# StanfordASL/RiskAverseTrajOpt

Hardware: AMD Instinct MI355X
Metric: SAA constraint-eval throughput (higher is better)
Workload: dtype f32

## Files before the change

### include/rato_saa.h

```cpp
#ifndef RATO_SAA_H
#define RATO_SAA_H

#include <stddef.h>
#include <stdint.h>

#ifdef __cplusplus
extern "C" {
#endif

#define RATO_OK 0
#define RATO_EINVAL (-1)
#define RATO_ENONFINITE (-2)
#define RATO_EINFEASIBLE (-4)
#define RATO_ENOCOMM (-3)
#define RATO_ERANK (-6)
#define RATO_ESELECT (-7)
#define RATO_ENNLS (-8)
#define RATO_EHIP (-1000)
#define RATO_ERCCL (-2000)

#define RATO_TILE 256
#define RATO_DRONE_NOBS 3
#define RATO_HOPPER_NFEAT 30

// ... 147 lines not shown
int rato_hopper_slip_host_inputs(int32_t M, int32_t C, const float* px_host, const float* fx_host,
                                 const float* fz_host, const float* a, const float* theta, const float* tau,
                                 const float* lam, float* Z, float* h, float* dh_dfz, float* dh_dpx,
                                 float* part_hess, void* stream);

int rato_hopper_slip_hessian(int32_t M, int32_t C, const float* px, const float* fx, const float* fz,
                             int32_t host_inputs, const float* a, const float* theta, const float* tau,
                             const float* lam, float* Z, float* h, float* dh_dfz, float* dh_dpx, float* part_hess3,
                             void* stream);

int64_t rato_hopper_jacobian_nnz(int32_t M, int32_t C, int32_t saa);
int rato_hopper_emit_jacobian_values(int32_t M, int32_t C, int32_t saa, double alpha, const float* dh_dfz,
                                     const float* dh_dpx, const float* chain_host, const float* chain_dev,
                                     int32_t write_constants, float* out, void* stream);


int rato_emit_csc_values(const float* G, const float* W ,
                         int64_t ld , int32_t tile, int32_t n_g, int32_t R, int32_t S,
                         int64_t M, float scale, float* out, void* stream);


int rato_saa_rowmax(const float* G, const float* W ,
                    int32_t tile, int32_t R, int32_t S, int64_t M, int64_t ld,
                    const float* base, double sign , const double* xs, int32_t n_u,
                    float* m_out, int32_t* arg_out, void* stream);

int rato_drone_rowmax_implicit(const rato_drone_params* p, const float* mass, const float* A22,
                               int32_t a22_axes ,
                               const float* W, const float* base, double sign, const double* xs,
                               float* m_out, int32_t* arg_out, void* stream);

int rato_drone_linearize_generators(const rato_drone_params* p, const float* us, const float* dW,
                                    const float* mass, const float* Qsym,
                                    float* A22, float* W, float* g_up, float* Z, float* part, void* stream);

int rato_saa_tail_rows_batch(const float* G, const float* W , int64_t ld, int32_t tile,
                             int32_t R, int32_t S, int64_t M, const float* base,
                             const float* m_base, const int32_t* arg_base, const double* stats_base,
                             int64_t stats_stride, const int32_t* slots, int32_t K, double alphaM, double* part,
                             void* stream);

int rato_drone_tail_rows_implicit(const rato_drone_params* p, const float* mass, const float* A22, int32_t a22_axes,
                                  const float* W, const float* base,
                                  const float* m_base, const int32_t* arg_base, const double* stats_base,
                                  int64_t stats_stride, const int32_t* slots, int32_t K, double alphaM,
                                  double* part, void* stream);

int rato_drone_rowmax_rollout(const rato_drone_params* p, const double* uk, const float* dW, const float* mass,
                              const float* Qsym, const double* xs, float* m_out, int32_t* arg_out, void* stream);
int rato_drone_tail_rows_rollout(const rato_drone_params* p, const double* uk, const float* dW, const float* mass,
                                 const float* Qsym, const float* m_base, const int32_t* arg_base,
                                 const double* stats_base, int64_t stats_stride, const int32_t* slots, int32_t K,
                                 double alphaM, double* part, void* stream);

int rato_car_rowmax_rollout(const rato_car_params* p, const double* uk, const float* dW, const float* x0_ped,
                            const float* w_speed, const float* w_rep, const double* xs, float* m_out,
                            int32_t* arg_out, void* stream);
int rato_car_tail_rows_rollout(const rato_car_params* p, const double* uk, const float* dW, const float* x0_ped,
                               const float* w_speed, const float* w_rep, const float* m_base, const int32_t* arg_base,
                               const double* stats_base, int64_t stats_stride, const int32_t* slots, int32_t K,
                               double alphaM, double* part, void* stream);

int rato_cut_oracle_rollout(int32_t system, const void* params, const double* uk, const float* s0, const float* s1,
                            const float* s2, const float* s3, const double* x_host, double* x_dev, float* m_out,
                            int32_t* arg_out, double alpha, float thr, double alphaM, void* workspace,
                            size_t workspace_bytes, double* res_dev, double* part_dev, double* res_host, void* stream);

int rato_kkt_sums(const float* m_star, int64_t M, const float* m_base, const double* stats_base, int64_t stats_stride,
                  const int32_t* slots, const double* lam, int32_t K, double alphaM, double v, double* part, void* stream);

typedef struct {
  int32_t system, S, cap, keep_max, keep_recent, keep_idle, mode_saa, recycle;
  int64_t M;
  double alpha, alphaM, c_s, rhs0, u_min, u_max;
  float thr;
  const void* params;
  const float *s0, *s1, *s2, *s3;
  double *uk_dev, *uk_host, *x_host, *x_dev;
  float* ring_m;
  int32_t* ring_arg;
  double* ring_res;
  void* workspace;
  size_t workspace_bytes;
  double *part, *part_b, *sums_b_host;
  int32_t *slots_dev, *slots_host;
  double* res_host;
  const double *p_diag, *q;
} rato_cut_config;

typedef struct {
  double* us;
  double slack, t_risk, phi, oracle_s, master_s, lam_slack;
  int32_t cuts, recycled, status, uncertified_cuts;
  int32_t* cut_slot;
  double* cut_lambda;
  int32_t cut_capacity, n_cut_rows;
  int32_t* bound_var;
  double* bound_sign;
  double* bound_lambda;
  int32_t bound_capacity, n_bounds;
} rato_cut_result;

typedef struct rato_cut_solver rato_cut_solver;
int rato_cut_solver_create(rato_cut_solver** out, const rato_cut_config* cfg);
void rato_cut_solver_destroy(rato_cut_solver* s);
size_t rato_cut_config_bytes(void);
// ... 281 lines not shown
```

### riskaversetrajopt_amd/_lib.py

```python
import ctypes as C
import os

from . import _build

_LIB = None
ABI_VERSION = 12

c_float_p = C.c_void_p
c_stream = C.c_void_p


class DroneParams(C.Structure):
    _fields_ = [("M", C.c_int32), ("ld", C.c_int32), ("S", C.c_int32), ("dt", C.c_float), ("beta", C.c_float),
                ("drag", C.c_float), ("kp", C.c_float), ("kd", C.c_float), ("tol", C.c_float),
                ("x_init", C.c_float * 6), ("x_final", C.c_float * 6),
                ("obs_xy", (C.c_float * 2) * 3), ("rows_out", C.c_int32),
                ("dt64", C.c_double), ("beta64", C.c_double), ("drag64", C.c_double), ("kp64", C.c_double),
                ("kd64", C.c_double), ("tol64", C.c_double), ("x_init64", C.c_double * 6),
                ("x_final64", C.c_double * 6), ("obs_xy64", (C.c_double * 2) * 3),
                ("stats_workspace", C.c_void_p), ("stats_out", C.c_void_p), ("stats_alpha", C.c_double),
                ("stats_thr", C.c_float), ("stats_flags", C.c_int32)]


class CarParams(C.Structure):
# ... 31 lines not shown
    _fields_ = [(k, C.c_int32) for k in ("n_tiles", "per_cu", "slots", "qslots", "wants_queue", "form", "split", "n_whole",
                                         "workgroups", "n_units")]


class CutConfig(C.Structure):
    _fields_ = [(k, C.c_int32) for k in ("system", "S", "cap", "keep_max", "keep_recent", "keep_idle", "mode_saa",
                                         "recycle")] + \
               [("M", C.c_int64)] + [(k, C.c_double) for k in ("alpha", "alphaM", "c_s", "rhs0", "u_min", "u_max")] + \
               [("thr", C.c_float), ("params", C.c_void_p)] + [(k, C.c_void_p) for k in ("s0", "s1", "s2", "s3")] + \
               [(k, C.c_void_p) for k in ("uk_dev", "uk_host", "x_host", "x_dev", "ring_m", "ring_arg", "ring_res",
                                          "workspace")] + [("workspace_bytes", C.c_size_t)] + \
               [(k, C.c_void_p) for k in ("part", "part_b", "sums_b_host", "slots_dev", "slots_host", "res_host",
                                          "p_diag", "q")]


class CutResult(C.Structure):
    _fields_ = [("us", C.c_void_p)] + \
               [(k, C.c_double) for k in ("slack", "t_risk", "phi", "oracle_s", "master_s", "lam_slack")] + \
               [(k, C.c_int32) for k in ("cuts", "recycled", "status", "uncertified_cuts")] + \
               [("cut_slot", C.c_void_p), ("cut_lambda", C.c_void_p), ("cut_capacity", C.c_int32),
                ("n_cut_rows", C.c_int32), ("bound_var", C.c_void_p), ("bound_sign", C.c_void_p),
                ("bound_lambda", C.c_void_p), ("bound_capacity", C.c_int32), ("n_bounds", C.c_int32)]


class ScpIter(C.Structure):
    _fields_ = [(k, C.c_double) for k in ("define_s", "solve_s", "oracle_s", "master_s", "t_risk", "slack", "phi")] + \
               [(k, C.c_int32) for k in ("cuts", "status", "recycled", "reserved")]


class ScpBatchIter(C.Structure):
    _fields_ = [(k, C.c_double) for k in ("define_s", "oracle_s", "master_s", "total_s")] + \
               [(k, C.c_int32) for k in ("rounds", "active", "reserved0", "reserved1")]


SIGNATURES = {
    "rato_abi_version": (C.c_int, []),
    "rato_packed_tile_stride": (C.c_size_t, [C.c_size_t]),
    "rato_packed_buffer_floats": (C.c_size_t, [C.c_size_t, C.c_size_t]),
    "rato_device_clock_probe": (C.c_int, [c_float_p, C.c_int32, c_stream]),
    "rato_device_occupy": (C.c_int, [C.c_int32, C.c_int64, c_stream]),
    "rato_drone_eval": (C.c_int, [C.POINTER(DroneParams)] + [c_float_p] * 7 + [c_stream]),
    "rato_drone_linearize_plan": (C.c_int, [C.c_int32, C.c_int32, C.c_int32, C.POINTER(C.c_int32),
                                            C.POINTER(C.c_int32), C.POINTER(C.c_int32)]),
    "rato_drone_linearize": (C.c_int, [C.POINTER(DroneParams)] + [c_float_p] * 10 + [C.c_int32, C.c_int32, c_stream]),
    "rato_drone_rowmax_implicit": (C.c_int, [C.POINTER(DroneParams), c_float_p, c_float_p, C.c_int32, c_float_p,
                                             c_float_p, C.c_double, c_float_p, c_float_p, c_float_p, c_stream]),
    "rato_drone_linearize_generators": (C.c_int, [C.POINTER(DroneParams)] + [c_float_p] * 9 + [c_stream]),
    "rato_drone_tail_rows_implicit": (C.c_int, [C.POINTER(DroneParams), c_float_p, c_float_p, C.c_int32] +
                                      [c_float_p] * 5 + [C.c_int64, c_float_p, C.c_int32, C.c_double, c_float_p,
                                                         c_stream]),
    "rato_drone_rowmax_rollout": (C.c_int, [C.POINTER(DroneParams)] + [c_float_p] * 7 + [c_stream]),
    "rato_drone_tail_rows_rollout": (C.c_int, [C.POINTER(DroneParams)] + [c_float_p] * 7 +
                                     [C.c_int64, c_float_p, C.c_int32, C.c_double, c_float_p, c_stream]),
    "rato_car_rowmax_rollout": (C.c_int, [C.POINTER(CarParams)] + [c_float_p] * 8 + [c_stream]),
    "rato_car_tail_rows_rollout": (C.c_int, [C.POINTER(CarParams)] + [c_float_p] * 8 +
                                   [C.c_int64, c_float_p, C.c_int32, C.c_double, c_float_p, c_stream]),
    "rato_cut_oracle_rollout": (C.c_int, [C.c_int32] + [c_float_p] * 10 + [C.c_double, C.c_float, C.c_double, C.c_void_p,
                                          C.c_size_t, c_float_p, c_float_p, c_float_p, c_stream]),
    "rato_kkt_sums": (C.c_int, [c_float_p, C.c_int64, c_float_p, c_float_p, C.c_int64, c_float_p, c_float_p, C.c_int32,
                                C.c_double, C.c_double, c_float_p, c_stream]),
    "rato_cut_solver_create": (C.c_int, [C.POINTER(C.c_void_p), C.POINTER(CutConfig)]),
    "rato_cut_solver_destroy": (None, [C.c_void_p]),
    "rato_cut_config_bytes": (C.c_size_t, []),
    "rato_cut_result_bytes": (C.c_size_t, []),
    "rato_cut_begin": (C.c_int, [C.c_void_p, C.c_void_p, C.c_void_p, C.c_int32, c_stream]),
    "rato_scp_iter_bytes": (C.c_size_t, []),
    "rato_scp_run_drone": (C.c_int, [C.c_void_p, C.c_void_p, C.c_int32, C.c_int32, C.c_double, C.c_int32, C.c_double, C.c_int32] +
                           [C.c_void_p] * 11 + [c_stream]),
    "rato_car_ego_final_rows": (C.c_int, [C.POINTER(CarParams), C.c_void_p, C.c_void_p, C.c_void_p, C.c_void_p]),
    "rato_scp_run_car": (C.c_int, [C.c_void_p, C.c_void_p, C.c_void_p, C.c_int32, C.c_int32, C.c_double, C.c_int32, C.c_double,
                                   C.c_int32] + [C.c_void_p] * 6 + [c_stream]),
    "rato_scp_batch_run_car": (C.c_int, [C.c_void_p, C.c_void_p, C.c_void_p, C.c_int32, C.c_int32, C.c_double, C.c_int32,
                                         C.c_double, C.c_int32] + [C.c_void_p] * 9 + [c_stream]),
    "rato_scp_batch_iter_bytes": (C.c_size_t, []),
    "rato_scp_batch_bytes": (C.c_int, [C.c_void_p, C.c_int32, C.POINTER(C.c_size_t), C.POINTER(C.c_size_t)]),
    "rato_scp_batch_create": (C.c_int, [C.POINTER(C.c_void_p), C.c_void_p, C.c_int32, C.c_int32, C.c_void_p, C.c_size_t,
                                        C.c_void_p, C.c_size_t]),
    "rato_scp_batch_destroy": (None, [C.c_void_p]),
    "rato_scp_batch_run_drone": (C.c_int, [C.c_void_p, C.c_void_p, C.c_int32, C.c_int32, C.c_double, C.c_int32, C.c_double,
                                           C.c_int32] + [C.c_void_p] * 9 + [c_stream]),
    "rato_cut_define_drone": (C.c_int, [C.c_void_p] * 6 + [C.c_int64] + [C.c_void_p] * 5 + [C.c_int32, c_stream]),
    "rato_cut_solve": (C.c_int, [C.c_void_p, C.c_void_p, C.c_void_p, C.c_int32, C.c_void_p, C.c_int32, C.c_double,
                                 C.c_int32, C.c_double, C.c_int32, C.c_void_p, C.c_void_p, C.POINTER(C.c_int32), C.c_int32,
                                 C.POINTER(CutResult), c_stream]),
    "rato_copy_async": (C.c_int, [C.c_void_p, C.c_void_p, C.c_size_t, c_stream]),
    "rato_stream_synchronize": (C.c_int, [c_stream]),
    "rato_master_create": (C.c_int, [C.POINTER(C.c_void_p), C.c_int32, C.c_void_p, C.c_void_p, C.c_int32, C.c_void_p,
                                     C.c_void_p]),
    "rato_master_add_rows": (C.c_int, [C.c_void_p, C.c_int32, C.c_void_p, C.c_void_p]),
    "rato_master_solve": (C.c_int, [C.c_void_p, C.c_void_p, C.c_void_p]),
    "rato_master_rows": (C.c_int32, [C.c_void_p]),
    "rato_master_destroy": (None, [C.c_void_p]),
    "rato_drone_obstacle_constraints": (C.c_int, [C.POINTER(DroneParams)] + [c_float_p] * 3 + [c_stream]),
    "rato_car_ego_scratch_floats": (C.c_size_t, [C.c_int32]),
    "rato_car_linearize_plan": (C.c_int, [C.c_int32, C.c_int32, C.POINTER(C.c_int32), C.POINTER(C.c_int32)]),
    "rato_car_eval": (C.c_int, [C.POINTER(CarParams)] + [c_float_p] * 9 + [c_stream]),
    "rato_car_separation_distances": (C.c_int, [C.POINTER(CarParams), c_float_p, c_float_p, c_stream]),
    "rato_car_linearize": (C.c_int, [C.POINTER(CarParams)] + [c_float_p] * 11 + [C.c_int32, c_stream]),
    "rato_hopper_nblocks": (C.c_int, [C.c_int32]),
    "rato_hopper_slip": (C.c_int, [C.c_int32, C.c_int32] + [c_float_p] * 12 + [c_stream]),
    "rato_hopper_slip_host_inputs": (C.c_int, [C.c_int32, C.c_int32] + [c_float_p] * 12 + [c_stream]),
    "rato_hopper_slip_hessian": (C.c_int, [C.c_int32, C.c_int32] + [c_float_p] * 3 + [C.c_int32] + [c_float_p] * 9 + [c_stream]),
    "rato_hopper_jacobian_nnz": (C.c_int64, [C.c_int32, C.c_int32, C.c_int32]),
    "rato_hopper_emit_jacobian_values": (C.c_int, [C.c_int32, C.c_int32, C.c_int32, C.c_double] + [c_float_p] * 4 +
                                         [C.c_int32, c_float_p, c_stream]),
    "rato_emit_csc_values": (C.c_int, [c_float_p, c_float_p, C.c_int64, C.c_int32, C.c_int32, C.c_int32, C.c_int32,
# ... 258 lines not shown
```

### riskaversetrajopt_amd/csrc/cvar.hip

```cpp
#include "rato_common.h"
#include <atomic>
#include <chrono>
#include <cstdlib>
#include <type_traits>

namespace {

constexpr int RM_NW = 8;

typedef double rdouble2_t __attribute__((ext_vector_type(2)));

__device__ __forceinline__ float tail_weight(float mv, float tstar, float lambda) {
  return (mv > tstar) ? 1.0f : ((mv == tstar) ? lambda : 0.0f);
}

__device__ __forceinline__ void tail_rule(const double* __restrict__ st, double alphaM, float& tstar, float& lambda) {
  tstar = (float)st[10];
  const double n_gt = st[8], n_eq = st[9];
  const double l = (n_eq > 0.0) ? (alphaM - n_gt) / n_eq : 0.0;
  lambda = (float)fmin(fmax(l, 0.0), 1.0);
}

__device__ __forceinline__ double a22_value(float stored, bool complement) {
  return complement ? 1.0 - (double)stored : (double)stored;
// ... 698 lines not shown
      w0f = tail_weight(mvals[m0], tstar, lambda);
      const int a = arg[m0];
      r0 = a / S;
      t0 = a - r0 * S;
    }
  }
  drone_tail_block(P, uk, dW, mass, Qsym, w0f, t0, r0, acc, E, Ctab);
#if RATO_TDIAG
  __syncthreads();
  if (threadIdx.x < 12) acc[threadIdx.x] = threadIdx.x == 10 ? (double)wall_clock64() : tdiag[threadIdx.x];
  __syncthreads();
#endif
  for (int i = threadIdx.x; i < nc; i += RATO_BLOCK) part[((size_t)blockIdx.x * K + kk) * nc + i] = acc[i];
}

__global__ __launch_bounds__(RATO_BLOCK) void drone_tail_rows_rollout_kernel(
    rato_drone_params P, const double* __restrict__ uk, const float* __restrict__ dW, const float* __restrict__ mass,
    const float* __restrict__ Qsym, const float* __restrict__ m_base, const int* __restrict__ arg_base,
    const double* __restrict__ stats_base, long stats_stride, const int* __restrict__ slots, double alphaM,
    double* __restrict__ part, int c_tab) {
  extern __shared__ __attribute__((aligned(16))) unsigned char trr_lds[];
  drone_tail_rows_rollout_block(P, uk, dW, mass, Qsym, m_base, arg_base, stats_base, stats_stride, slots, alphaM, part, c_tab,
                                gridDim.y, blockIdx.y, trr_lds);
}

__global__ __launch_bounds__(RATO_BLOCK) void drone_tail_rows_rollout_batch_kernel(rato_drone_params P,
                                                                                   const rato::BatchProb* __restrict__ tab,
                                                                                   long stats_stride, int c_tab) {
  extern __shared__ __attribute__((aligned(16))) unsigned char trr_lds[];
  const rato::BatchProb& t = tab[blockIdx.y];
  drone_tail_rows_rollout_block(P, t.uk, t.s0, t.s1, t.s2, t.m_out, t.arg_out, t.res_dev, stats_stride, nullptr,
                                t.alphaM, t.part, c_tab, 1, 0, trr_lds);
}

__global__ __launch_bounds__(RATO_BLOCK) void drone_tail_rows_rollout_kept_batch_kernel(
    rato_drone_params P, const rato::BatchProb* __restrict__ tab, const rato::BatchCut* __restrict__ rows, long stats_stride,
    int c_tab) {
  extern __shared__ __attribute__((aligned(16))) unsigned char trr_lds[];
  const rato::BatchCut r = rows[blockIdx.y];
  const rato::BatchProb& t = tab[r.prob];
  drone_tail_rows_rollout_block(P, t.uk, t.s0, t.s1, t.s2, t.m_base, t.arg_base, t.res_base, stats_stride, t.slots,
                                t.alphaM, t.part_b, c_tab, r.K, r.k0, trr_lds);
}

#ifndef RATO_TRU_NW
#define RATO_TRU_NW 8
#endif
constexpr int TRU_NW = RATO_TRU_NW, TRU_KMAX = 16;
__host__ __device__ inline size_t tail_union_lds_bytes(int S, int K) {
  const size_t nc = 2 * (size_t)(S - 1) + 1;
  return sizeof(double) * ((size_t)K * nc + (size_t)K * 2 * RATO_WAVE) + sizeof(float) * (size_t)S * 2 * RATO_WAVE +
         (sizeof(float) + sizeof(int)) * (size_t)K * RATO_WAVE + sizeof(unsigned) * (size_t)S;
}
__device__ __forceinline__ void drone_tail_rows_rollout_union_block(
    const rato_drone_params& P, const double* __restrict__ uk, const float* __restrict__ dW, const float* __restrict__ mass,
    const float* __restrict__ Qsym, const float* __restrict__ m_base, const int* __restrict__ arg_base,
    const double* __restrict__ stats_base, long stats_stride, const int* __restrict__ slots, int k0, int K, int K_total,
    double alphaM, double* __restrict__ part, unsigned char* tru_lds) {
  constexpr int NT = TRU_NW * RATO_WAVE;
  const int S = P.S;
  const long M = P.M, ld = P.ld;
  const int nw = 2 * (S - 1), nc = nw + 1;
  double* acc = reinterpret_cast<double*>(tru_lds);
  double* GW = acc + (size_t)K * nc;
  float* E = reinterpret_cast<float*>(GW + (size_t)K * 2 * RATO_WAVE);
  float* WT = E + (size_t)S * 2 * RATO_WAVE;
  int* TR = reinterpret_cast<int*>(WT + (size_t)K * RATO_WAVE);
  unsigned* TMASK = reinterpret_cast<unsigned*>(TR + (size_t)K * RATO_WAVE);
  __shared__ int s_src[RATO_BLOCK];
  __shared__ int s_cnt[RATO_BLOCK / RATO_WAVE];
  __shared__ float s_ts[TRU_KMAX], s_lam[TRU_KMAX];
  __shared__ long s_slot[TRU_KMAX];
  const int tid = threadIdx.x, lane = tid & 63, wave = tid >> 6;
  const long block_base = (long)blockIdx.x * RATO_BLOCK;
  if (tid < K) {
    const long slot = slots[k0 + tid];
    float ts, lam;
    tail_rule(stats_base + slot * stats_stride, alphaM, ts, lam);
    s_ts[tid] = ts;
    s_lam[tid] = lam;
    s_slot[tid] = slot;
  }
  for (int i = tid; i < K * nc; i += NT) acc[i] = 0.0;
  __syncthreads();
  bool act = false;
  if (tid < RATO_BLOCK && block_base + tid < M) {
    for (int kk = 0; kk < K; ++kk)
      act = act || (tail_weight(m_base[s_slot[kk] * M + block_base + tid], s_ts[kk], s_lam[kk]) != 0.0f);
  }
  const unsigned long long bal = __ballot(act);
  if (wave < RATO_BLOCK / RATO_WAVE && lane == 0) s_cnt[wave] = __popcll(bal);
  __syncthreads();
  int base = 0, n_un = 0;
#pragma unroll
  for (int i = 0; i < RATO_BLOCK / RATO_WAVE; ++i) {
    const int c = s_cnt[i];
    if (i < wave) base += c;
    n_un += c;
  }
  if (act) s_src[base + __popcll(bal & ((1ull << lane) - 1ull))] = tid;
  const double dt = P.dt64, kp = P.kp64, kd = P.kd64, drag = P.drag64;
  for (int c0 = 0; c0 < n_un; c0 += RATO_WAVE) {
    for (int i = tid; i < S; i += NT) TMASK[i] = 0u;
    __syncthreads();
    for (int idx = tid; idx < K * RATO_WAVE; idx += NT) {
      const int kk = idx >> 6, l = idx & 63;
      float w = 0.0f;
      int tr = 0;
      if (c0 + l < n_un) {
        const long m = block_base + s_src[c0 + l];
        w = tail_weight(m_base[s_slot[kk] * M + m], s_ts[kk], s_lam[kk]);
        const int a = arg_base[s_slot[kk] * M + m];
        const int r = a / S, t = a - r * S;
        tr = t | (r << 20);
        if (w != 0.0f) atomicOr(&TMASK[t], 1u << kk);
      }
      WT[idx] = w;
      TR[idx] = tr;
    }
    __syncthreads();
    const bool on = c0 + lane < n_un;
    const long m = on ? block_base + s_src[c0 + lane] : block_base;
    const double inv_m = 1.0 / (double)mass[m];
    const double a21 = -kp * dt * inv_m, dtm = dt * inv_m;
    if (wave == 0) {
      const double cn = sqrt(dt) * P.beta64 * inv_m;
      const double c1 = dt * kd * inv_m, one_c1 = 1.0 - c1, c2 = dt * drag * inv_m, c22 = 2.0 * c2;
      int t_hi = 0;
      {
        int tm = 0;
        for (int kk = 0; kk < K; ++kk)
          if (WT[kk * RATO_WAVE + lane] != 0.0f) tm = max(tm, TR[kk * RATO_WAVE + lane] & 0xfffff);
#pragma unroll
        for (int off = 32; off > 0; off >>= 1) tm = max(tm, __shfl_xor(tm, off, RATO_WAVE));
        t_hi = __builtin_amdgcn_readfirstlane(tm);
      }
      double p[2] = {P.x_init64[0], P.x_init64[1]}, v[2] = {P.x_init64[3], P.x_init64[4]};
      constexpr int TB = 8;
      auto load = [&](float (&xi)[TB][2], int tb) {
#pragma unroll
        for (int i = 0; i < TB; ++i) {
          const int t = (tb + i <= t_hi) ? tb + i : t_hi;
          xi[i][0] = dW[((size_t)t * 3 + 0) * ld + m];
          xi[i][1] = dW[((size_t)t * 3 + 1) * ld + m];
        }
      };
      auto steps = [&](const float (&xi)[TB][2], int tb) {
#pragma unroll
        for (int i = 0; i < TB; ++i) {
          const int t = tb + i;
          if (t <= t_hi) {
#pragma unroll
            for (int a = 0; a < 2; ++a) {
              const double av = fabs(v[a]);
              E[(t * 2 + a) * RATO_WAVE + lane] = (float)fma(c22, av, c1);
              const double tv = fma(a21, p[a], fma(dtm, uk[t * 3 + a], cn * (double)xi[i][a]));
              const double pn = fma(dt, v[a], p[a]);
              v[a] = fma(fma(-c2, av, one_c1), v[a], tv);
              p[a] = pn;
            }
            unsigned mask = __builtin_amdgcn_readfirstlane(TMASK[t]);
            while (mask) {
              const int kk = __builtin_ctz(mask);
              mask &= mask - 1u;
              if (on && WT[kk * RATO_WAVE + lane] != 0.0f && (TR[kk * RATO_WAVE + lane] & 0xfffff) == t) {
                GW[(kk * 2 + 0) * RATO_WAVE + lane] = p[0];
                GW[(kk * 2 + 1) * RATO_WAVE + lane] = p[1];
              }
            }
          }
        }
      };
      float xa[TB][2], xb[TB][2];
      load(xa, 0);
      for (int tb = 0; tb <= t_hi; tb += 2 * TB) {
        load(xb, tb + TB);
        steps(xa, tb);
        load(xa, tb + 2 * TB);
        steps(xb, tb + TB);
      }
    }
    __syncthreads();
    for (int kk = wave; kk < K; kk += TRU_NW) {
      const float wf = WT[kk * RATO_WAVE + lane];
      const bool in_tail = on && wf != 0.0f;
      const int ts = in_tail ? (TR[kk * RATO_WAVE + lane] & 0xfffff) : 0;
      const double w = in_tail ? (double)wf : 0.0;
      double gval = 0.0, w0 = 0.0, w1 = 0.0;
      if (in_tail) {
        const int rs = TR[kk * RATO_WAVE + lane] >> 20;
        const double q00 = (double)Qsym[(size_t)(rs * 3 + 0) * ld + m], qss = (double)Qsym[(size_t)(rs * 3 + 1) * ld + m],
                     q11 = (double)Qsym[(size_t)(rs * 3 + 2) * ld + m];
        const double ox = rs == 0 ? P.obs_xy64[0][0] : (rs == 1 ? P.obs_xy64[1][0] : P.obs_xy64[2][0]);
        const double oy = rs == 0 ? P.obs_xy64[0][1] : (rs == 1 ? P.obs_xy64[1][1] : P.obs_xy64[2][1]);
        const double dx = GW[(kk * 2 + 0) * RATO_WAVE + lane] - ox, dy = GW[(kk * 2 + 1) * RATO_WAVE + lane] - oy;
        gval = 1.0 - (q00 * dx * dx + qss * dx * dy + q11 * dy * dy);
        w0 = w * -(2.0 * q00 * dx + qss * dy) * dtm;
        w1 = w * -(qss * dx + 2.0 * q11 * dy) * dtm;
      }
      int t_hi = 0;
      {
        int tm = ts;
#pragma unroll
        for (int off = 32; off > 0; off >>= 1) tm = max(tm, __shfl_xor(tm, off, RATO_WAVE));
        t_hi = __builtin_amdgcn_readfirstlane(tm);
      }
      double* __restrict__ ak = acc + (size_t)kk * nc;
      const bool cols_in_regs = S - 1 <= RATO_WAVE;
      double colx = 0.0, coly = 0.0;
      double m0x = 0.0, m1x = 0.0, m0y = 0.0, m1y = 0.0;
      for (int k = t_hi; k >= 1; --k) {
        const bool in = in_tail && k <= ts;
        if (in && k == ts) {
          m0x = 1.0; m1x = 0.0; m0y = 1.0; m1y = 0.0;
        }
        double cx = 0.0, cy = 0.0;
        if (in) {
          const double ax = 1.0 - (double)E[(k * 2 + 0) * RATO_WAVE + lane], ay = 1.0 - (double)E[(k * 2 + 1) * RATO_WAVE + lane];
          const double n0x = m0x + m1x * a21, n1x = m0x * dt + m1x * ax;
          const double n0y = m0y + m1y * a21, n1y = m0y * dt + m1y * ay;
          m0x = n0x; m1x = n1x; m0y = n0y; m1y = n1y;
          cx = w0 * m1x;
          cy = w1 * m1y;
        }
        const double s0 = rato::wave_sum_dpp(cx);
        const double s1 = rato::wave_sum_dpp(cy);
        if (cols_in_regs) {
          colx += (lane == k - 1) ? s0 : 0.0;
          coly += (lane == k - 1) ? s1 : 0.0;
        } else if (lane == 0) {
          ak[(k - 1) * 2 + 0] += s0;
          ak[(k - 1) * 2 + 1] += s1;
        }
      }
      if (cols_in_regs && lane < S - 1) {
        ak[lane * 2 + 0] += colx;
        ak[lane * 2 + 1] += coly;
      }
      const double sg = rato::wave_sum_dpp(w * gval);
      if (lane == 0) ak[nw] += sg;
    }
  }
  __syncthreads();
  for (int i = tid; i < K * nc; i += NT) {
    const int kk = i / nc, j = i - kk * nc;
    part[((size_t)blockIdx.x * K_total + (k0 + kk)) * nc + j] = acc[i];
  }
}

__global__ __launch_bounds__(TRU_NW* RATO_WAVE) void drone_tail_rows_rollout_union_kernel(
    rato_drone_params P, const double* __restrict__ uk, const float* __restrict__ dW, const float* __restrict__ mass,
    const float* __restrict__ Qsym, const float* __restrict__ m_base, const int* __restrict__ arg_base,
    const double* __restrict__ stats_base, long stats_stride, const int* __restrict__ slots, int k0, int K, int K_total,
    double alphaM, double* __restrict__ part) {
  extern __shared__ __attribute__((aligned(16))) unsigned char tru_lds[];
  drone_tail_rows_rollout_union_block(P, uk, dW, mass, Qsym, m_base, arg_base, stats_base, stats_stride, slots, k0, K, K_total,
                                      alphaM, part, tru_lds);
}

__global__ __launch_bounds__(TRU_NW* RATO_WAVE) void drone_tail_rows_rollout_union_batch_kernel(
    rato_drone_params P, const rato::BatchProb* __restrict__ tab, const rato::BatchCut* __restrict__ rows, long stats_stride) {
  extern __shared__ __attribute__((aligned(16))) unsigned char tru_lds[];
  const rato::BatchCut r = rows[blockIdx.y];
  const rato::BatchProb& t = tab[r.prob];
  drone_tail_rows_rollout_union_block(P, t.uk, t.s0, t.s1, t.s2, t.m_base, t.arg_base, t.res_base, stats_stride, t.slots,
                                      r.k0, r.kn, r.K, t.alphaM, t.part_b, tru_lds);
}

template <bool TANGENT>
__device__ __forceinline__ void car_ego64_tables(const rato_car_params& P, const double* __restrict__ uk,
                                                 const double* __restrict__ xs, double* U ,
                                                 double* TERM , double* EGO ,
                                                 double* AUX ) {
  const int S = P.S;
  const double dt = P.dt64;
  for (int i = threadIdx.x; i < 2 * S; i += blockDim.x) {
    U[i] = uk[i];
    if (TANGENT) U[2 * S + i] = xs[i];
  }
  __syncthreads();
  for (int t = threadIdx.x; t <= S; t += blockDim.x) {
    double v = P.ego_init64[2], ph = P.ego_init64[3], dv = 0.0, dph = 0.0;
    for (int k = 0; k < t; ++k) {
      v += dt * U[2 * k + 0];
      ph += dt * U[2 * k + 1];
      if (TANGENT) {
        dv += dt * U[2 * S + 2 * k + 0];
        dph += dt * U[2 * S + 2 * k + 1];
      }
    }
    double sn, cs;
    sincos(ph, &sn, &cs);
    TERM[t * 4 + 0] = dt * v * cs;
    TERM[t * 4 + 1] = dt * v * sn;
    if (TANGENT) {
      TERM[t * 4 + 2] = dt * (dv * cs - v * sn * dph);
      TERM[t * 4 + 3] = dt * (dv * sn + v * cs * dph);
    } else if (t < S) {
      AUX[t * 4 + 0] = -dt * dt * cs;
      AUX[t * 4 + 1] = dt * dt * v * sn;
      AUX[t * 4 + 2] = -dt * dt * sn;
      AUX[t * 4 + 3] = -dt * dt * v * cs;
    }
  }
  __syncthreads();
  for (int t = threadIdx.x; t <= S; t += blockDim.x) {
    double x = P.ego_init64[0], y = P.ego_init64[1], dx = 0.0, dy = 0.0;
    for (int k = 0; k < t; ++k) {
      x += TERM[k * 4 + 0];
      y += TERM[k * 4 + 1];
      if (TANGENT) {
        dx += TERM[k * 4 + 2];
        dy += TERM[k * 4 + 3];
      }
    }
    EGO[t * 2 + 0] = x;
    EGO[t * 2 + 1] = y;
    if (TANGENT) {
      AUX[t * 2 + 0] = dx;
// ... 366 lines not shown
                                             int64_t stats_stride, const int32_t* slots, int32_t K, double alphaM,
                                             double* part, void* stream) {
  RATO_CLEAR_ERROR();
  if (!p || p->M <= 0 || p->S < 2 || p->ld < p->M || !(p->dt > 0.0f) || !(p->dt64 > 0.0) || !mass || !A22 || !W || !base || !m_base ||
      !arg_base || !stats_base || !part || K < 1 || K > 65535 || (!slots && K != 1) || stats_stride < 11 ||
      (a22_axes != 2 && a22_axes != 3))
    return RATO_EINVAL;
  const size_t lds = (size_t)(RATO_BLOCK / 64) * (2 * (p->S - 1) + 1) * sizeof(double);
  dim3 grid((unsigned)rato::nblocks_for(p->M), (unsigned)K), block(RATO_BLOCK);
  hipLaunchKernelGGL(drone_tail_rows_implicit_kernel, grid, block, lds, rato::as_stream(stream), *p, mass, A22,
                     a22_axes, W, base, m_base, arg_base, stats_base, (long)stats_stride, slots, alphaM, part);
  RATO_LAUNCH_CHECK();
  return RATO_OK;
}

extern "C" int rato_saa_tail_rows_batch(const float* G, const float* W, int64_t ld, int32_t tile, int32_t R, int32_t S,
                                        int64_t M, const float* base, const float* m_base, const int32_t* arg_base,
                                        const double* stats_base, int64_t stats_stride, const int32_t* slots,
                                        int32_t K, double alphaM, double* part, void* stream) {
  RATO_CLEAR_ERROR();
  if (!G || !base || !m_base || !arg_base || !stats_base || !part || M <= 0 || S < 2 || K < 1 || K > 65535 ||
      (!slots && K != 1) || ld < M || stats_stride < 11 || (tile != 64 && tile != 256) || (R != 1 && R != 3))
    return RATO_EINVAL;
  const size_t lds = (size_t)(RATO_BLOCK / 64) * (2 * (S - 1) + 1) * sizeof(double);
  dim3 grid((unsigned)rato::nblocks_for((int32_t)M), (unsigned)K), block(RATO_BLOCK);
  hipStream_t st = rato::as_stream(stream);
  if (R == 3)
    hipLaunchKernelGGL(tail_rows_batch_kernel<3>, grid, block, lds, st, G, W, (long)ld, tile, S, (long)M, base, m_base,
                       arg_base, stats_base, (long)stats_stride, slots, alphaM, part);
  else
    hipLaunchKernelGGL(tail_rows_batch_kernel<1>, grid, block, lds, st, G, W, (long)ld, tile, S, (long)M, base, m_base,
                       arg_base, stats_base, (long)stats_stride, slots, alphaM, part);
  RATO_LAUNCH_CHECK();
  return RATO_OK;
}

namespace {
size_t tail_rows_lds(int S, int& c_tab) {
  const size_t lds = (size_t)(2 * (S - 1) + 1) * sizeof(double) + (size_t)S * 2 * RATO_WAVE * sizeof(float);
  c_tab = 0;
  if (lds + 4096 > 160 * 1024) return 0;
  static const int ctab_env = [] { const char* e = getenv("RATO_TAIL_CTAB"); return e ? atoi(e) : 1; }();
  const size_t lds_c = lds + tail_ctab_doubles(S) * sizeof(double);
  c_tab = (ctab_env && lds_c + 4096 <= 80 * 1024) ? 1 : 0;
  return c_tab ? lds_c : lds;
}
}

namespace rato {
bool drone_tail_union_form(int S, int K) {
  static const int union_env = [] { const char* e = getenv("RATO_TAIL_UNION"); return e ? atoi(e) : 1; }();
  return K > 1 && union_env && tail_union_lds_bytes(S, K < TRU_KMAX ? K : TRU_KMAX) + 4096 <= 160 * 1024;
}
}

namespace {
int drone_rowmax_rollout_launch(const rato_drone_params* p, const double* uk, const float* dW, const float* mass,
                                const float* Qsym, const double* xs, const double* xs_host, float* m_out,
                                int32_t* arg_out, void* stream) {
  RATO_CLEAR_ERROR();
  if (!p || p->M <= 0 || p->S < 1 || p->ld < p->M || !(p->dt > 0.0f) || !(p->dt64 > 0.0) || !uk || !dW || !mass || !Qsym ||
      (!xs && !xs_host) || !m_out || !arg_out)
    return RATO_EINVAL;
  dim3 grid((unsigned)rato::nblocks_for(p->M)), block(RATO_BLOCK);
  XArg xv;
  if (xs_host && p->S * 3 <= XARG_MAX) {
    for (int i = 0; i < p->S * 3; ++i) xv.v[i] = xs_host[i];
    hipLaunchKernelGGL(drone_rowmax_rollout_kernel<true>, grid, block, 0, rato::as_stream(stream), *p, uk, dW, mass, Qsym,
                       xs, xv, m_out, arg_out);
  } else {
    if (!xs) return RATO_EINVAL;
    hipLaunchKernelGGL(drone_rowmax_rollout_kernel<false>, grid, block, 0, rato::as_stream(stream), *p, uk, dW, mass, Qsym,
                       xs, xv, m_out, arg_out);
  }
  RATO_LAUNCH_CHECK();
  return RATO_OK;
}
}

extern "C" int rato_drone_rowmax_rollout(const rato_drone_params* p, const double* uk, const float* dW,
                                         const float* mass, const float* Qsym, const double* xs, float* m_out,
                                         int32_t* arg_out, void* stream) {
  if (!xs) return RATO_EINVAL;
  return drone_rowmax_rollout_launch(p, uk, dW, mass, Qsym, xs, nullptr, m_out, arg_out, stream);
}

extern "C" int rato_drone_tail_rows_rollout(const rato_drone_params* p, const double* uk, const float* dW,
                                            const float* mass, const float* Qsym, const float* m_base,
                                            const int32_t* arg_base, const double* stats_base, int64_t stats_stride,
                                            const int32_t* slots, int32_t K, double alphaM, double* part,
                                            void* stream) {
  RATO_CLEAR_ERROR();
  if (!p || p->M <= 0 || p->S < 2 || p->S >= (1 << 20) || p->ld < p->M || !(p->dt > 0.0f) || !(p->dt64 > 0.0) || !uk || !dW || !mass ||
      !Qsym || !m_base || !arg_base || !stats_base || !part || K < 1 || K > 65535 || (!slots && K != 1) ||
      stats_stride < 11)
    return RATO_EINVAL;
  int c_tab = 0;
  const size_t lds = tail_rows_lds(p->S, c_tab);
  if (!lds) return RATO_EINVAL;
  if (rato::drone_tail_union_form(p->S, K)) {
    static rato::DynamicLdsLimit lds_limit_u;
    for (int k0 = 0; k0 < K; k0 += TRU_KMAX) {
      const int kn = (K - k0) < TRU_KMAX ? (K - k0) : TRU_KMAX;
      const size_t lds_u = tail_union_lds_bytes(p->S, kn);
      const int rc = rato::launch_dynamic_lds(drone_tail_rows_rollout_union_kernel, lds_limit_u, lds_u, lds_u,
                                              dim3((unsigned)rato::nblocks_for(p->M)), dim3(TRU_NW * RATO_WAVE),
                                              rato::as_stream(stream), *p, uk, dW, mass, Qsym, m_base, arg_base, stats_base,
                                              (long)stats_stride, slots, k0, kn, K, alphaM, part);
      if (rc != RATO_OK) return rc;
    }
    return RATO_OK;
  }
  static rato::DynamicLdsLimit lds_limit;
  dim3 grid((unsigned)rato::nblocks_for(p->M), (unsigned)K), block(RATO_BLOCK);
  return rato::launch_dynamic_lds(drone_tail_rows_rollout_kernel, lds_limit, lds, lds, grid, block, rato::as_stream(stream), *p,
                                  uk, dW, mass, Qsym, m_base, arg_base, stats_base, (long)stats_stride, slots, alphaM, part,
                                  c_tab);
}


namespace rato {
int launch_drone_rowmax_rollout_batch(const rato_drone_params* p, const BatchProb* tab, int n, hipStream_t st) {
  RATO_CLEAR_ERROR();
  if (!p || !tab || n < 1 || n > 65535) return RATO_EINVAL;
  hipLaunchKernelGGL(drone_rowmax_rollout_batch_kernel, dim3((unsigned)rato::nblocks_for(p->M), (unsigned)n), dim3(RATO_BLOCK), 0,
                     st, *p, tab);
  RATO_LAUNCH_CHECK();
  return RATO_OK;
}

int launch_drone_tail_rows_batch(const rato_drone_params* p, const BatchProb* tab, int n, hipStream_t st) {
  RATO_CLEAR_ERROR();
  if (!p || !tab || n < 1 || n > 65535 || p->S < 2) return RATO_EINVAL;
  int c_tab = 0;
  const size_t lds = tail_rows_lds(p->S, c_tab);
  if (!lds) return RATO_EINVAL;
  static rato::DynamicLdsLimit lds_limit;
  return launch_dynamic_lds(drone_tail_rows_rollout_batch_kernel, lds_limit, lds, lds,
                            dim3((unsigned)rato::nblocks_for(p->M), (unsigned)n), dim3(RATO_BLOCK), st, *p, tab,
                            (long)record_words(p->S), c_tab);
}

int launch_drone_tail_kept_batch(const rato_drone_params* p, const BatchProb* tab, const BatchCut* rows, int n_rows,
                                 bool union_form, int kn_max, hipStream_t st) {
  RATO_CLEAR_ERROR();
  if (!p || !tab || !rows || n_rows < 1 || n_rows > 65535 || p->S < 2 || kn_max < 1 || kn_max > TRU_KMAX) return RATO_EINVAL;
  const long stride = record_words(p->S);
  const dim3 grid((unsigned)rato::nblocks_for(p->M), (unsigned)n_rows);
  if (union_form) {
    const size_t lds_u = tail_union_lds_bytes(p->S, kn_max);
    static rato::DynamicLdsLimit lds_limit_u;
    return launch_dynamic_lds(drone_tail_rows_rollout_union_batch_kernel, lds_limit_u, lds_u, lds_u, grid,
                              dim3(TRU_NW * RATO_WAVE), st, *p, tab, rows, stride);
  }
  int c_tab = 0;
  const size_t lds = tail_rows_lds(p->S, c_tab);
  if (!lds) return RATO_EINVAL;
  static rato::DynamicLdsLimit lds_limit;
  return launch_dynamic_lds(drone_tail_rows_rollout_kept_batch_kernel, lds_limit, lds, lds, grid, dim3(RATO_BLOCK), st, *p, tab,
                            rows, stride, c_tab);
}
}

namespace {
bool car_params64_ok(const rato_car_params* p) {
  return p && p->M > 0 && p->S >= 1 && p->S <= 1024 && p->dt64 > 0.0 && p->d_min64 >= 0.0;
}
size_t car_tail_rows_lds(int S) {
  return (car_rollout_ego_doubles(S) + (size_t)(2 * (S - 1) + 1)) * sizeof(double) + (size_t)S * 3 * RATO_WAVE * sizeof(float);
}
}

namespace {
int car_rowmax_rollout_launch(const rato_car_params* p, const double* uk, const float* dW, const float* x0_ped,
                              const float* w_speed, const float* w_rep, const double* xs, const double* xs_host,
                              float* m_out, int32_t* arg_out, void* stream) {
  RATO_CLEAR_ERROR();
  if (!car_params64_ok(p) || !uk || !dW || !x0_ped || !w_speed || !w_rep || (!xs && !xs_host) || !m_out || !arg_out)
    return RATO_EINVAL;
  const size_t lds = car_rollout_ego_doubles(p->S) * sizeof(double);
  if (lds > 64 * 1024) return RATO_EINVAL;
  dim3 grid((unsigned)rato::nblocks_for(p->M)), block(RATO_BLOCK);
  XArg xv;
  if (xs_host && p->S * 2 <= XARG_MAX) {
    for (int i = 0; i < p->S * 2; ++i) xv.v[i] = xs_host[i];
    hipLaunchKernelGGL(car_rowmax_rollout_kernel<true>, grid, block, lds, rato::as_stream(stream), *p, uk, dW, x0_ped,
                       w_speed, w_rep, xs, xv, m_out, arg_out);
  } else {
    if (!xs) return RATO_EINVAL;
    hipLaunchKernelGGL(car_rowmax_rollout_kernel<false>, grid, block, lds, rato::as_stream(stream), *p, uk, dW, x0_ped,
                       w_speed, w_rep, xs, xv, m_out, arg_out);
  }
  RATO_LAUNCH_CHECK();
  return RATO_OK;
}
}

extern "C" int rato_car_rowmax_rollout(const rato_car_params* p, const double* uk, const float* dW,
                                       const float* x0_ped, const float* w_speed, const float* w_rep,
                                       const double* xs, float* m_out, int32_t* arg_out, void* stream) {
  if (!xs) return RATO_EINVAL;
  return car_rowmax_rollout_launch(p, uk, dW, x0_ped, w_speed, w_rep, xs, nullptr, m_out, arg_out, stream);
}

extern "C" int rato_car_tail_rows_rollout(const rato_car_params* p, const double* uk, const float* dW,
// ... 117 lines not shown
```

### riskaversetrajopt_amd/csrc/rato_common.h

```cpp
#pragma once
#include <hip/hip_runtime.h>
#include <stdint.h>
#include <stdio.h>
#include <stdlib.h>

#include <atomic>
#include <chrono>
#include <mutex>

#include "rato_saa.h"

#if defined(__HIP_DEVICE_COMPILE__) && !defined(__gfx950__)
#error "librato_saa is written for gfx950 (MI355X) only: see the hardware assumptions in rato_common.h"
#endif

#define RATO_BLOCK 256
#define RATO_WAVE 64

#define RATO_CLEAR_ERROR() (void)hipGetLastError()

#define RATO_LAUNCH_CHECK()                              \
  do {                                                   \
    hipError_t e__ = hipGetLastError();                  \
    if (e__ != hipSuccess) return RATO_EHIP - (int)e__;  \
// ... 150 lines not shown
    std::lock_guard<std::mutex> lock(mu_);
    PerDev& d = dev_[dev];
    if (d.cus == 0) {
      int n = 256;
      (void)hipDeviceGetAttribute(&n, hipDeviceAttributeMultiprocessorCount, dev);
      d.cus = n > 0 ? n : 256;
    }
    return d.cus;
  }

 private:
  static constexpr int kMaxDev = 32;
  struct PerDev {
    unsigned* base = nullptr;
    hipStream_t owner[RATO_QUEUES_EAGER] = {};
    int used = 0, next_captured = RATO_QUEUES_EAGER, cus = 0;
    bool warned = false;
  };
  std::mutex mu_;
  PerDev dev_[kMaxDev];
};

int launch_cut_finish(const double* part, int nblocks, int ncols, double* rec_dev, double* rec_host, int n_stats,
                      hipStream_t st);

struct BatchProb {
  const double* uk;
  const float *s0, *s1, *s2, *s3;
  const double* x;
  const float* us;
  float *A22, *gpart;
  double* sums_host;
  const int32_t* slots;
  int32_t n_keep;
  uint32_t k;
  int32_t var_is_max;
  float thr;
  double alpha, alphaM;
  const float* m_base;
  const int32_t* arg_base;
  const double* res_base;
  float* m_out;
  int32_t* arg_out;
  double *res_dev, *res_host, *part;
  double *part_b, *sums_b_host;
};
inline int record_words(int S) { return RATO_N_STATS + 2 * (S - 1) + 1; }
struct BatchCut {
  int32_t prob, k0, kn, K;
};
int launch_drone_rowmax_rollout_batch(const rato_drone_params* p, const BatchProb* tab, int n, hipStream_t st);
int launch_drone_tail_rows_batch(const rato_drone_params* p, const BatchProb* tab, int n, hipStream_t st);
bool drone_tail_union_form(int S, int K);
int launch_drone_tail_kept_batch(const rato_drone_params* p, const BatchProb* tab, const BatchCut* rows, int n_rows,
                                 bool union_form, int kn_max, hipStream_t st);
int launch_car_rowmax_rollout_batch(const rato_car_params* p, const BatchProb* tab, int n, hipStream_t st);
int launch_car_tail_rows_batch(const rato_car_params* p, const BatchProb* tab, int n, hipStream_t st);
int launch_car_tail_kept_batch(const rato_car_params* p, const BatchProb* tab, const BatchCut* rows, int n_rows,
                               hipStream_t st);
bool risk_stats_batch_applies(int64_t M);
int launch_risk_stats_batch(const BatchProb* tab, int n, int64_t M, hipStream_t st);
int launch_cut_finish_batch(const BatchProb* tab, int n, int nblocks, int ncols, int n_stats, hipStream_t st);
int launch_define_sums_batch(const BatchProb* tab, int n, int nblocks, int ncols, hipStream_t st);
int launch_kept_sums_batch(const BatchProb* tab, int n, int nblocks, int nc, int max_keep, hipStream_t st);
int launch_drone_linearize_generators_batch(const rato_drone_params* p, const BatchProb* tab, int n, hipStream_t st);

constexpr uint64_t READBACK_PENDING = 0x7ff8dead5a5abeefull;
inline bool readback_poll_enabled() {
  static const int v = [] { const char* e = getenv("RATO_CUT_POLL"); return e ? atoi(e) : 1; }();
  return v != 0;
}
inline void readback_arm(double* host, int n) {
  volatile uint64_t* w = reinterpret_cast<volatile uint64_t*>(host);
  for (int i = 0; i < n; ++i) w[i] = READBACK_PENDING;
}
inline bool readback_pending(const double* host, int n) {
  const volatile uint64_t* w = reinterpret_cast<const volatile uint64_t*>(host);
  for (int i = 0; i < n; ++i)
    if (w[i] == READBACK_PENDING) return true;
  return false;
}
inline hipError_t readback_wait(const double* host, int n, hipStream_t st) {
  if (readback_poll_enabled()) {
    const volatile uint64_t* w = reinterpret_cast<const volatile uint64_t*>(host);
    const auto t0 = std::chrono::steady_clock::now();
    for (unsigned spins = 0;; ++spins) {
      int pending = 0;
      for (int i = 0; i < n; ++i) pending += w[i] == READBACK_PENDING;
      if (!pending) {
        std::atomic_thread_fence(std::memory_order_acquire);
        return hipSuccess;
      }
      __builtin_ia32_pause();
      if ((spins & 0xfff) == 0xfff && std::chrono::steady_clock::now() - t0 > std::chrono::seconds(2)) break;
    }
  }
  const hipError_t e = hipStreamSynchronize(st);
  if (e != hipSuccess || !readback_poll_enabled()) return e;
  return readback_pending(host, n) ? hipErrorNotReady : hipSuccess;
}

class DynamicLdsLimit {
 public:
  template <class Apply>
  hipError_t ensure(size_t bytes, Apply&& apply) {
    if (bytes <= 64 * 1024) return hipSuccess;
// ... 29 lines not shown
```

Before: 9.813 billion.

## Split drone tail-union rollout across two waves and per-axis adjoint tasks

```diff
diff --git a/include/rato_saa.h b/include/rato_saa.h
--- a/include/rato_saa.h
+++ b/include/rato_saa.h
@@ -223,6 +223,7 @@
                                  const float* Qsym, const float* m_base, const int32_t* arg_base,
                                  const double* stats_base, int64_t stats_stride, const int32_t* slots, int32_t K,
                                  double alphaM, double* part, void* stream);
+int rato_drone_tail_rows_form(int32_t S, int32_t K);
 
 int rato_car_rowmax_rollout(const rato_car_params* p, const double* uk, const float* dW, const float* x0_ped,
                             const float* w_speed, const float* w_rep, const double* xs, float* m_out,
diff --git a/riskaversetrajopt_amd/_lib.py b/riskaversetrajopt_amd/_lib.py
--- a/riskaversetrajopt_amd/_lib.py
+++ b/riskaversetrajopt_amd/_lib.py
@@ -107,6 +107,7 @@
     "rato_drone_rowmax_rollout": (C.c_int, [C.POINTER(DroneParams)] + [c_float_p] * 7 + [c_stream]),
     "rato_drone_tail_rows_rollout": (C.c_int, [C.POINTER(DroneParams)] + [c_float_p] * 7 +
                                      [C.c_int64, c_float_p, C.c_int32, C.c_double, c_float_p, c_stream]),
+    "rato_drone_tail_rows_form": (C.c_int, [C.c_int32, C.c_int32]),
     "rato_car_rowmax_rollout": (C.c_int, [C.POINTER(CarParams)] + [c_float_p] * 8 + [c_stream]),
     "rato_car_tail_rows_rollout": (C.c_int, [C.POINTER(CarParams)] + [c_float_p] * 8 +
                                    [C.c_int64, c_float_p, C.c_int32, C.c_double, c_float_p, c_stream]),
diff --git a/riskaversetrajopt_amd/csrc/cvar.hip b/riskaversetrajopt_amd/csrc/cvar.hip
--- a/riskaversetrajopt_amd/csrc/cvar.hip
+++ b/riskaversetrajopt_amd/csrc/cvar.hip
@@ -774,6 +774,9 @@
   return sizeof(double) * ((size_t)K * nc + (size_t)K * 2 * RATO_WAVE) + sizeof(float) * (size_t)S * 2 * RATO_WAVE +
          (sizeof(float) + sizeof(int)) * (size_t)K * RATO_WAVE + sizeof(unsigned) * (size_t)S;
 }
+__host__ __device__ inline size_t tail_union_park_offset(int S, int K) { return (tail_union_lds_bytes(S, K) + 15) & ~(size_t)15; }
+__host__ __device__ inline size_t tail_union_park_bytes() { return sizeof(double) * (size_t)TRU_NW * 4 * RATO_WAVE; }
+template <bool SPLIT>
 __device__ __forceinline__ void drone_tail_rows_rollout_union_block(
     const rato_drone_params& P, const double* __restrict__ uk, const float* __restrict__ dW, const float* __restrict__ mass,
     const float* __restrict__ Qsym, const float* __restrict__ m_base, const int* __restrict__ arg_base,
@@ -807,8 +810,17 @@
   __syncthreads();
   bool act = false;
   if (tid < RATO_BLOCK && block_base + tid < M) {
-    for (int kk = 0; kk < K; ++kk)
-      act = act || (tail_weight(m_base[s_slot[kk] * M + block_base + tid], s_ts[kk], s_lam[kk]) != 0.0f);
+    if constexpr (SPLIT) {
+      float mv[TRU_KMAX];
+#pragma unroll
+      for (int kk = 0; kk < TRU_KMAX; ++kk) mv[kk] = m_base[s_slot[kk < K ? kk : K - 1] * M + block_base + tid];
+#pragma unroll
+      for (int kk = 0; kk < TRU_KMAX; ++kk)
+        if (kk < K) act = act | (tail_weight(mv[kk], s_ts[kk], s_lam[kk]) != 0.0f);
+    } else {
+      for (int kk = 0; kk < K; ++kk)
+        act = act || (tail_weight(m_base[s_slot[kk] * M + block_base + tid], s_ts[kk], s_lam[kk]) != 0.0f);
+    }
   }
   const unsigned long long bal = __ballot(act);
   if (wave < RATO_BLOCK / RATO_WAVE && lane == 0) s_cnt[wave] = __popcll(bal);
@@ -825,6 +837,38 @@
   for (int c0 = 0; c0 < n_un; c0 += RATO_WAVE) {
     for (int i = tid; i < S; i += NT) TMASK[i] = 0u;
     __syncthreads();
+    if constexpr (SPLIT) {
+      static_assert(TRU_KMAX * RATO_WAVE <= 2 * NT, "two entries per thread cover the table");
+      float mv[2] = {0.0f, 0.0f};
+      int av[2] = {0, 0};
+      bool ld_on[2];
+#pragma unroll
+      for (int j = 0; j < 2; ++j) {
+        const int idx = tid + j * NT, kk = idx >> 6, l = idx & 63;
+        ld_on[j] = idx < K * RATO_WAVE && c0 + l < n_un;
+        if (ld_on[j]) {
+          const long m = block_base + s_src[c0 + l];
+          mv[j] = m_base[s_slot[kk] * M + m];
+          av[j] = arg_base[s_slot[kk] * M + m];
+        }
+      }
+#pragma unroll
+      for (int j = 0; j < 2; ++j) {
+        const int idx = tid + j * NT, kk = idx >> 6;
+        if (idx < K * RATO_WAVE) {
+          float w = 0.0f;
+          int tr = 0;
+          if (ld_on[j]) {
+            w = tail_weight(mv[j], s_ts[kk], s_lam[kk]);
+            const int r = av[j] / S, t = av[j] - r * S;
+            tr = t | (r << 20);
+            if (w != 0.0f) atomicOr(&TMASK[t], 1u << kk);
+          }
+          WT[idx] = w;
+          TR[idx] = tr;
+        }
+      }
+    } else {
     for (int idx = tid; idx < K * RATO_WAVE; idx += NT) {
       const int kk = idx >> 6, l = idx & 63;
       float w = 0.0f;
@@ -840,12 +884,66 @@
       WT[idx] = w;
       TR[idx] = tr;
     }
+    }
     __syncthreads();
     const bool on = c0 + lane < n_un;
     const long m = on ? block_base + s_src[c0 + lane] : block_base;
     const double inv_m = 1.0 / (double)mass[m];
     const double a21 = -kp * dt * inv_m, dtm = dt * inv_m;
-    if (wave == 0) {
+    if (SPLIT && wave < 2) {
+      const int a = wave;
+      const double cn = sqrt(dt) * P.beta64 * inv_m;
+      const double c1 = dt * kd * inv_m, one_c1 = 1.0 - c1, c2 = dt * drag * inv_m, c22 = 2.0 * c2;
+      int t_hi = 0;
+      {
+        int tm = 0;
+        for (int kk = 0; kk < K; ++kk)
+          if (WT[kk * RATO_WAVE + lane] != 0.0f) tm = max(tm, TR[kk * RATO_WAVE + lane] & 0xfffff);
+#pragma unroll
+        for (int off = 32; off > 0; off >>= 1) tm = max(tm, __shfl_xor(tm, off, RATO_WAVE));
+        t_hi = __builtin_amdgcn_readfirstlane(tm);
+      }
+      double p = a == 0 ? P.x_init64[0] : P.x_init64[1], v = a == 0 ? P.x_init64[3] : P.x_init64[4];
+      constexpr int TB = 8;
+      const float* __restrict__ dWa = dW + (size_t)a * ld + m;
+      auto load = [&](float (&xi)[TB], int tb) {
+#pragma unroll
+        for (int i = 0; i < TB; ++i) {
+          const int t = (tb + i <= t_hi) ? tb + i : t_hi;
+          xi[i] = dWa[(size_t)t * 3 * ld];
+        }
+      };
+      auto steps = [&](const float (&xi)[TB], int tb) {
+#pragma unroll
+        for (int i = 0; i < TB; ++i) {
+          const int t = tb + i;
+          if (t <= t_hi) {
+            const double av = fabs(v);
+            E[(t * 2 + a) * RATO_WAVE + lane] = (float)fma(c22, av, c1);
+            const double tv = fma(a21, p, fma(dtm, uk[t * 3 + a], cn * (double)xi[i]));
+            const double pn = fma(dt, v, p);
+            v = fma(fma(-c2, av, one_c1), v, tv);
+            p = pn;
+            unsigned mask = __builtin_amdgcn_readfirstlane(TMASK[t]);
+            while (mask) {
+              const int kk = __builtin_ctz(mask);
+              mask &= mask - 1u;
+              if (on && WT[kk * RATO_WAVE + lane] != 0.0f && (TR[kk * RATO_WAVE + lane] & 0xfffff) == t)
+                GW[(kk * 2 + a) * RATO_WAVE + lane] = p;
+            }
+          }
+        }
+      };
+      float xa[TB], xb[TB];
+      load(xa, 0);
+      for (int tb = 0; tb <= t_hi; tb += 2 * TB) {
+        load(xb, tb + TB);
+        steps(xa, tb);
+        load(xa, tb + 2 * TB);
+        steps(xb, tb + TB);
+      }
+    }
+    if (!SPLIT && wave == 0) {
       const double cn = sqrt(dt) * P.beta64 * inv_m;
       const double c1 = dt * kd * inv_m, one_c1 = 1.0 - c1, c2 = dt * drag * inv_m, c22 = 2.0 * c2;
       int t_hi = 0;
@@ -903,7 +1001,8 @@
       }
     }
     __syncthreads();
-    for (int kk = wave; kk < K; kk += TRU_NW) {
+    for (int task = wave; SPLIT && task < 2 * K; task += TRU_NW) {
+      const int kk = task >> 1, ax = task & 1;
       const float wf = WT[kk * RATO_WAVE + lane];
       const bool in_tail = on && wf != 0.0f;
       const int ts = in_tail ? (TR[kk * RATO_WAVE + lane] & 0xfffff) : 0;
@@ -920,6 +1019,64 @@
         w0 = w * -(2.0 * q00 * dx + qss * dy) * dtm;
         w1 = w * -(qss * dx + 2.0 * q11 * dy) * dtm;
       }
+      const double wa = ax == 0 ? w0 : w1;
+      int t_hi = 0;
+      {
+        int tm = ts;
+#pragma unroll
+        for (int off = 32; off > 0; off >>= 1) tm = max(tm, __shfl_xor(tm, off, RATO_WAVE));
+        t_hi = __builtin_amdgcn_readfirstlane(tm);
+      }
+      double* __restrict__ ak = acc + (size_t)kk * nc;
+      double* const Tp = reinterpret_cast<double*>(tru_lds + tail_union_park_offset(S, K)) + wave * (4 * RATO_WAVE);
+      double m0 = 0.0, m1 = 0.0;
+      for (int kq = t_hi; kq >= 1; kq -= 4) {
+#pragma unroll
+        for (int r = 0; r < 4; ++r) {
+          const int k = kq - r;
+          if (k >= 1) {
+            const bool in = in_tail && k <= ts;
+            if (in && k == ts) {
+              m0 = 1.0; m1 = 0.0;
+            }
+            double c = 0.0;
+            if (in) {
+              const double aa = 1.0 - (double)E[(k * 2 + ax) * RATO_WAVE + lane];
+              const double n0 = m0 + m1 * a21, n1 = m0 * dt + m1 * aa;
+              m0 = n0; m1 = n1;
+              c = wa * m1;
+            }
+            Tp[r * RATO_WAVE + lane] = c;
+          }
+        }
+        const double* src = Tp + (lane >> 4) * RATO_WAVE + (lane & 15) * 4;
+        const double y = (src[1] + src[0]) + (src[3] + src[2]);
+        const double s0 = rato::row16_sum_dpp(y);
+        const int k = kq - (lane >> 4);
+        if ((lane & 15) == 15 && k >= 1) ak[(k - 1) * 2 + ax] += s0;
+      }
+      if (ax == 0) {
+        const double sg = rato::wave_sum_dpp(w * gval);
+        if (lane == 0) ak[nw] += sg;
+      }
+    }
+    for (int kk = wave; !SPLIT && kk < K; kk += TRU_NW) {
+      const float wf = WT[kk * RATO_WAVE + lane];
+      const bool in_tail = on && wf != 0.0f;
+      const int ts = in_tail ? (TR[kk * RATO_WAVE + lane] & 0xfffff) : 0;
+      const double w = in_tail ? (double)wf : 0.0;
+      double gval = 0.0, w0 = 0.0, w1 = 0.0;
+      if (in_tail) {
+        const int rs = TR[kk * RATO_WAVE + lane] >> 20;
+        const double q00 = (double)Qsym[(size_t)(rs * 3 + 0) * ld + m], qss = (double)Qsym[(size_t)(rs * 3 + 1) * ld + m],
+                     q11 = (double)Qsym[(size_t)(rs * 3 + 2) * ld + m];
+        const double ox = rs == 0 ? P.obs_xy64[0][0] : (rs == 1 ? P.obs_xy64[1][0] : P.obs_xy64[2][0]);
+        const double oy = rs == 0 ? P.obs_xy64[0][1] : (rs == 1 ? P.obs_xy64[1][1] : P.obs_xy64[2][1]);
+        const double dx = GW[(kk * 2 + 0) * RATO_WAVE + lane] - ox, dy = GW[(kk * 2 + 1) * RATO_WAVE + lane] - oy;
+        gval = 1.0 - (q00 * dx * dx + qss * dx * dy + q11 * dy * dy);
+        w0 = w * -(2.0 * q00 * dx + qss * dy) * dtm;
+        w1 = w * -(qss * dx + 2.0 * q11 * dy) * dtm;
+      }
       int t_hi = 0;
       {
         int tm = ts;
@@ -970,23 +1127,25 @@
   }
 }
 
+template <bool SPLIT>
 __global__ __launch_bounds__(TRU_NW* RATO_WAVE) void drone_tail_rows_rollout_union_kernel(
     rato_drone_params P, const double* __restrict__ uk, const float* __restrict__ dW, const float* __restrict__ mass,
     const float* __restrict__ Qsym, const float* __restrict__ m_base, const int* __restrict__ arg_base,
     const double* __restrict__ stats_base, long stats_stride, const int* __restrict__ slots, int k0, int K, int K_total,
     double alphaM, double* __restrict__ part) {
   extern __shared__ __attribute__((aligned(16))) unsigned char tru_lds[];
-  drone_tail_rows_rollout_union_block(P, uk, dW, mass, Qsym, m_base, arg_base, stats_base, stats_stride, slots, k0, K, K_total,
-                                      alphaM, part, tru_lds);
-}
-
+  drone_tail_rows_rollout_union_block<SPLIT>(P, uk, dW, mass, Qsym, m_base, arg_base, stats_base, stats_stride, slots, k0, K,
+                                             K_total, alphaM, part, tru_lds);
+}
+
+template <bool SPLIT>
 __global__ __launch_bounds__(TRU_NW* RATO_WAVE) void drone_tail_rows_rollout_union_batch_kernel(
     rato_drone_params P, const rato::BatchProb* __restrict__ tab, const rato::BatchCut* __restrict__ rows, long stats_stride) {
   extern __shared__ __attribute__((aligned(16))) unsigned char tru_lds[];
   const rato::BatchCut r = rows[blockIdx.y];
   const rato::BatchProb& t = tab[r.prob];
-  drone_tail_rows_rollout_union_block(P, t.uk, t.s0, t.s1, t.s2, t.m_base, t.arg_base, t.res_base, stats_stride, t.slots,
-                                      r.k0, r.kn, r.K, t.alphaM, t.part_b, tru_lds);
+  drone_tail_rows_rollout_union_block<SPLIT>(P, t.uk, t.s0, t.s1, t.s2, t.m_base, t.arg_base, t.res_base, stats_stride,
+                                             t.slots, r.k0, r.kn, r.K, t.alphaM, t.part_b, tru_lds);
 }
 
 template <bool TANGENT>
@@ -1459,6 +1618,16 @@
   static const int union_env = [] { const char* e = getenv("RATO_TAIL_UNION"); return e ? atoi(e) : 1; }();
   return K > 1 && union_env && tail_union_lds_bytes(S, K < TRU_KMAX ? K : TRU_KMAX) + 4096 <= 160 * 1024;
 }
+bool drone_tail_union_split(int S, int K) {
+  static const int split_env = [] { const char* e = getenv("RATO_TAIL_UNION_SPLIT"); return e ? atoi(e) : 1; }();
+  return split_env && K <= TRU_KMAX && drone_tail_union_form(S, K) &&
+         tail_union_park_offset(S, K) + tail_union_park_bytes() + 4096 <= 160 * 1024;
+}
+}
+
+extern "C" int rato_drone_tail_rows_form(int32_t S, int32_t K) {
+  if (S < 2 || K < 1) return RATO_EINVAL;
+  return rato::drone_tail_union_split(S, K) ? 2 : (rato::drone_tail_union_form(S, K) ? 1 : 0);
 }
 
 namespace {
@@ -1506,11 +1675,19 @@
   const size_t lds = tail_rows_lds(p->S, c_tab);
   if (!lds) return RATO_EINVAL;
   if (rato::drone_tail_union_form(p->S, K)) {
+    if (rato::drone_tail_union_split(p->S, K)) {
+      static rato::DynamicLdsLimit lds_limit_s;
+      const size_t lds_s = tail_union_park_offset(p->S, K) + tail_union_park_bytes();
+      return rato::launch_dynamic_lds(drone_tail_rows_rollout_union_kernel<true>, lds_limit_s, lds_s, lds_s,
+                                      dim3((unsigned)rato::nblocks_for(p->M)), dim3(TRU_NW * RATO_WAVE),
+                                      rato::as_stream(stream), *p, uk, dW, mass, Qsym, m_base, arg_base, stats_base,
+                                      (long)stats_stride, slots, 0, K, K, alphaM, part);
+    }
     static rato::DynamicLdsLimit lds_limit_u;
     for (int k0 = 0; k0 < K; k0 += TRU_KMAX) {
       const int kn = (K - k0) < TRU_KMAX ? (K - k0) : TRU_KMAX;
       const size_t lds_u = tail_union_lds_bytes(p->S, kn);
-      const int rc = rato::launch_dynamic_lds(drone_tail_rows_rollout_union_kernel, lds_limit_u, lds_u, lds_u,
+      const int rc = rato::launch_dynamic_lds(drone_tail_rows_rollout_union_kernel<false>, lds_limit_u, lds_u, lds_u,
                                               dim3((unsigned)rato::nblocks_for(p->M)), dim3(TRU_NW * RATO_WAVE),
                                               rato::as_stream(stream), *p, uk, dW, mass, Qsym, m_base, arg_base, stats_base,
                                               (long)stats_stride, slots, k0, kn, K, alphaM, part);
@@ -1556,8 +1733,14 @@
   const dim3 grid((unsigned)rato::nblocks_for(p->M), (unsigned)n_rows);
   if (union_form) {
     const size_t lds_u = tail_union_lds_bytes(p->S, kn_max);
+    if (drone_tail_union_split(p->S, kn_max)) {
+      static rato::DynamicLdsLimit lds_limit_s;
+      const size_t lds_s = tail_union_park_offset(p->S, kn_max) + tail_union_park_bytes();
+      return launch_dynamic_lds(drone_tail_rows_rollout_union_batch_kernel<true>, lds_limit_s, lds_s, lds_s, grid,
+                                dim3(TRU_NW * RATO_WAVE), st, *p, tab, rows, stride);
+    }
     static rato::DynamicLdsLimit lds_limit_u;
-    return launch_dynamic_lds(drone_tail_rows_rollout_union_batch_kernel, lds_limit_u, lds_u, lds_u, grid,
+    return launch_dynamic_lds(drone_tail_rows_rollout_union_batch_kernel<false>, lds_limit_u, lds_u, lds_u, grid,
                               dim3(TRU_NW * RATO_WAVE), st, *p, tab, rows, stride);
   }
   int c_tab = 0;
diff --git a/riskaversetrajopt_amd/csrc/rato_common.h b/riskaversetrajopt_amd/csrc/rato_common.h
--- a/riskaversetrajopt_amd/csrc/rato_common.h
+++ b/riskaversetrajopt_amd/csrc/rato_common.h
@@ -226,6 +226,7 @@
 int launch_drone_rowmax_rollout_batch(const rato_drone_params* p, const BatchProb* tab, int n, hipStream_t st);
 int launch_drone_tail_rows_batch(const rato_drone_params* p, const BatchProb* tab, int n, hipStream_t st);
 bool drone_tail_union_form(int S, int K);
+bool drone_tail_union_split(int S, int K);
 int launch_drone_tail_kept_batch(const rato_drone_params* p, const BatchProb* tab, const BatchCut* rows, int n_rows,
                                  bool union_form, int kn_max, hipStream_t st);
 int launch_car_rowmax_rollout_batch(const rato_car_params* p, const BatchProb* tab, int n, hipStream_t st);
```

Result: slower. 9.664 billion (-1.5%).
